# tyiannak/pyAudioAnalysis

Measured on AMD Instinct MI355X. Metric: short-term frames/sec (34-feat, 16 kHz, 50 ms/25 ms) + HBM GB/s vs peak, higher is better.
Workload: dtype f64

## Files before the change

### pyaudioanalysis_amd/csrc/device_common.hpp

```cpp
#pragma once
#include <float.h>
#include <hip/hip_runtime.h>
#include <stdint.h>

namespace paa {

constexpr int kWave = 64;
constexpr int kBase = 34;
constexpr int kFlush = 8;
constexpr double kEps = 2.220446049250313e-16;
#ifdef PAA_EXPERIMENTS
#define PAA_DEBUG_BIT(word, bit) (((word) & (bit)) != 0)
#else
#define PAA_DEBUG_BIT(word, bit) false
#endif

struct ClipDev {
    long long sample_off;
    long long n;
    long long out_off;
    int T;
    int stat_first;
    int stat_count;
    int pad;
// ... 173 lines not shown
    return v;
}
__device__ __forceinline__ int group_min_i(int v) {
    v = min(v, dpp_mov_i<PAA_DPP_X1>(v));
    v = min(v, dpp_mov_i<PAA_DPP_X2>(v));
    v = min(v, dpp_mov_i<PAA_DPP_HM>(v));
    v = min(v, dpp_mov_i<PAA_DPP_RM>(v));
    return v;
}
__device__ __forceinline__ double group_scan_incl(double v) {
    v += dpp_mov<0x111>(v);
    v += dpp_mov<0x112>(v);
    v += dpp_mov<0x114>(v);
    v += dpp_mov<0x118>(v);
    return v;
}

__device__ __forceinline__ void wsync() {
    asm volatile("" ::: "memory");
    __builtin_amdgcn_wave_barrier();
    asm volatile("" ::: "memory");
}


__device__ __forceinline__ double readlane63(double v) {
    const int lo = __builtin_amdgcn_readlane(__double2loint(v), 63);
    const int hi = __builtin_amdgcn_readlane(__double2hiint(v), 63);
    return __hiloint2double(hi, lo);
}
template <int CTRL, int ROWMASK>
__device__ __forceinline__ double dpp_mov_rows(double v) {
    int lo = __builtin_amdgcn_update_dpp(0, __double2loint(v), CTRL, ROWMASK, 0xF, false);
    int hi = __builtin_amdgcn_update_dpp(0, __double2hiint(v), CTRL, ROWMASK, 0xF, false);
    return __hiloint2double(hi, lo);
}
__device__ __forceinline__ double wsum(double v) {
    v = group_sum(v);
    v += dpp_mov_rows<0x142, 0xA>(v);
    v += dpp_mov_rows<0x143, 0xC>(v);
    return readlane63(v);
}
__device__ __forceinline__ double wmax_nonneg(double v) {
    v = group_max(v);
    v = fmax(v, dpp_mov_rows<0x142, 0xA>(v));
    v = fmax(v, dpp_mov_rows<0x143, 0xC>(v));
    return readlane63(v);
}
__device__ __forceinline__ int wsum_i(int v) {
    v = group_sum_i(v);
    v += __builtin_amdgcn_update_dpp(0, v, 0x142, 0xA, 0xF, false);
    v += __builtin_amdgcn_update_dpp(0, v, 0x143, 0xC, 0xF, false);
    return __builtin_amdgcn_readlane(v, 63);
}
__device__ __forceinline__ int wmin_i(int v) {
#pragma unroll
    for (int o = 32; o > 0; o >>= 1) v = min(v, __shfl_xor(v, o, 64));
    return v;
}
__device__ __forceinline__ double wscan_incl(double v) {
    v = group_scan_incl(v);
    v += dpp_mov_rows<0x142, 0xA>(v);
    v += dpp_mov_rows<0x143, 0xC>(v);
    return v;
}

__device__ __forceinline__ double fast_sqrt(double x) {
    const double y = __builtin_amdgcn_rsq(x);
    double g = x * y;
    double h = 0.5 * y;
    const double r = fma(-h, g, 0.5);
    g = fma(g, r, g);
    h = fma(h, r, h);
    const double d = fma(-g, g, x);
    g = fma(d, h, g);
    return (x > 0.0) ? g : 0.0;
}
__device__ __forceinline__ double mag_sqrt(double x) {
    const unsigned hi_ = max((unsigned)__double2hiint(x), 0x01a56e1fu);
    const double y = __builtin_amdgcn_rsq(__hiloint2double((int)hi_, __double2loint(x)));
    const double g = x * y;
    const double h = 0.5 * y;
    const double r = fma(-h, g, 0.5);
    return fma(g, r, g);
}

__device__ __forceinline__ double fast_div(double a, double b) {
    double r = __builtin_amdgcn_rcp(b);
    r = fma(fma(-b, r, 1.0), r, r);
    r = fma(fma(-b, r, 1.0), r, r);
    const double q = a * r;
    return fma(fma(-b, q, a), r, q);
}

__device__ __forceinline__ double fast_log2(double x) {
    double m = __builtin_amdgcn_frexp_mant(x);
    int e = __builtin_amdgcn_frexp_exp(x);
    const bool lo = m < 0.70710678118654752440;
    m = lo ? m + m : m;
    e = lo ? e - 1 : e;
    const double num = m - 1.0, den = m + 1.0;
    double r = __builtin_amdgcn_rcp(den);
    r = fma(fma(-den, r, 1.0), r, r);
    r = fma(fma(-den, r, 1.0), r, r);
    double s = num * r;
    s = fma(fma(-den, s, num), r, s);
    const double z = s * s;
    double p = 1.0 / 21.0;
    p = fma(p, z, 1.0 / 19.0);
    p = fma(p, z, 1.0 / 17.0);
    p = fma(p, z, 1.0 / 15.0);
    p = fma(p, z, 1.0 / 13.0);
    p = fma(p, z, 1.0 / 11.0);
    p = fma(p, z, 1.0 / 9.0);
    p = fma(p, z, 1.0 / 7.0);
    p = fma(p, z, 1.0 / 5.0);
    p = fma(p, z, 1.0 / 3.0);
    p = fma(p, z, 1.0);
    return fma(s * p, 2.8853900817779268147, (double)e);
}
__device__ __forceinline__ double fast_log10(double x) { return fast_log2(x) * 0.30102999566398119521; }

template <typename T> __device__ __forceinline__ double load_sample(const T *p);
template <> __device__ __forceinline__ double load_sample<int16_t>(const int16_t *p) { return (double)(*p); }
template <> __device__ __forceinline__ double load_sample<double>(const double *p) { return *p; }
struct alignas(4) stereo16 { int16_t l, r; };
__device__ __forceinline__ int stereo_word_sum(int w) { return (int)(short)(w & 0xffff) + (w >> 16); }
template <> __device__ __forceinline__ double load_sample<stereo16>(const stereo16 *p) {
    return (double)stereo_word_sum(*reinterpret_cast<const int *>(p));
}
template <typename T> __host__ __device__ constexpr double sample_scale() { return 1.0 / 32768.0; }
template <> __host__ __device__ constexpr double sample_scale<stereo16>() { return 1.0 / 65536.0; }

struct SignRule {
    int zb1, lo, sh;
};
__device__ __forceinline__ int sgn1(int x, const SignRule &q) {
    int t;
    asm("v_med3_i32 %0, %1, %2, 2" : "=v"(t) : "v"(x - q.zb1), "v"(q.lo));
    return t;
}
__device__ __forceinline__ int sgn1(double d) { return ((d > 0.0) ? 2 : 1) - ((d < 0.0) ? 1 : 0); }
__device__ __forceinline__ void sad_acc(int &acc, int a, int b) { asm("v_sad_u32 %0, %1, %2, %0" : "+v"(acc) : "v"(a), "v"(b)); }
template <typename T>
__device__ __forceinline__ SignRule sign_rule(double mean) {
    const double thr = mean * (1.0 / sample_scale<T>());
    const double fl = floor(thr);
    const bool whole = (fl == thr);
    SignRule q;
    q.zb1 = (int)fl - 1;
    q.lo = whole ? 0 : 1;
    q.sh = __builtin_amdgcn_readfirstlane(whole ? 0 : 1);
    asm volatile("" : "+v"(q.zb1), "+v"(q.lo));
    return q;
}

template <typename SumT, typename MmT>
__device__ __forceinline__ ClipNorm clip_norm_wave(const ClipDev &cd, const SumT *__restrict__ psum,
                                                   const MmT *__restrict__ pmin, const MmT *__restrict__ pmax, double sc,
                                                   int window, int lane) {
    SumT s = 0;
    double mn = DBL_MAX, mx = -DBL_MAX;
    const SumT *ps = psum + cd.stat_first;
    const MmT *pn = pmin + cd.stat_first, *px = pmax + cd.stat_first;
    int i = lane;
    for (; i + 192 < cd.stat_count; i += 256) {
        SumT a[4];
// ... 65 lines not shown
```

### pyaudioanalysis_amd/csrc/kernels_fast.hpp

```cpp
#pragma once
#include <algorithm>
#include <vector>

#include "device_common.hpp"
#include "tables.hpp"

namespace paa {

struct FastTables {
    void *d_blob = nullptr;
};
namespace f800 {
struct TabLayout {
    int off_w0, off_k0, off_w1, off_k1, off_w2, off_k2;
    int off_chw, off_chk;
    int off_dct;
    int off_tw2, off_twp;
    int off_sync;
    int melN0, melN1, melN2, chN;
    int mel_clamp;
    double f0, rf0, r_half_fs, f0sq;
    int fixed_lists;
    int pace_mode;
    int total;
// ... 24 lines not shown
constexpr int CH_STRIDE = 12;

template <int S, int NW = 4>
struct Geo {
    static_assert(S % CHUNK == 0 && S % 8 == 0, "step must be a multiple of the 40-sample chunk");
    static constexpr int RAW_N = (QUAD - 1) * S + W;
    static constexpr int NCHUNK = RAW_N / CHUNK;
    static constexpr int CPF = S / CHUNK;
    static constexpr int NPRE = (RAW_N / 8 + 63) / 64;
    static constexpr int PAD = (NW == 8 && S == 800) ? 0 : RAW_PAD;
    static constexpr int RAW_BYTES = (RAW_N + 2 * PAD) * 2;
    static constexpr bool ALIAS = (NW == 8);
    static constexpr int OFF_SPEC = 0;
    static constexpr int OFF_RAW = OFF_SPEC + 5 * NF * 8;
    static constexpr int OFF_CE = ALIAS ? OFF_RAW : OFF_RAW + RAW_BYTES;
    static constexpr int OFF_CZ = OFF_CE + NCHUNK * 8;
    static constexpr int OFF_FV = OFF_CZ + 2 * NCHUNK * 4;
    static constexpr int LDS_BYTES = ALIAS ? OFF_FV : OFF_FV + QUAD * FV_STRIDE * 8;
    static constexpr int WAVE_BYTES = ((LDS_BYTES + 15) / 16) * 16;
    static_assert(OFF_RAW % 16 == 0 && OFF_CE % 8 == 0 && OFF_FV % 8 == 0, "LDS alignment");
    static_assert(QUAD * 40 * 8 <= RAW_BYTES, "msp alias fits in the raw buffer");
    static_assert(!ALIAS || RAW_BYTES <= 2 * NF * 8, "raw[] fits in two spectrum slots");
    static_assert(!ALIAS || QUAD * 40 * 8 + QUAD * FV_STRIDE * 8 <= NF * 8, "msp + fv fit in one spectrum slot");
};

__device__ __forceinline__ void dft5r(double2 &a0, double2 &a1, double2 &a2, double2 &a3, double2 &a4) {
    const double c1 = 0.30901699437494742410;
    const double s1 = 0.95105651629515357212, s2 = 0.58778525229247312917;
    const double2 t1 = cadd(a1, a4), t2 = cadd(a2, a3), t3 = csub(a1, a4), t4 = csub(a2, a3);
    const double2 d = csub(t1, t2);
    const double2 h1 = make_double2(fma(-0.5, t1.x, a0.x), fma(-0.5, t1.y, a0.y));
    const double2 h2 = make_double2(fma(-0.5, t2.x, a0.x), fma(-0.5, t2.y, a0.y));
    const double2 m1 = make_double2(fma(c1, d.x, h2.x), fma(c1, d.y, h2.y));
    const double2 m2 = make_double2(fma(-c1, d.x, h1.x), fma(-c1, d.y, h1.y));
    const double2 n1 = make_double2(fma(s2, t4.x, s1 * t3.x), fma(s2, t4.y, s1 * t3.y));
    const double2 n2 = make_double2(fma(-s1, t4.x, s2 * t3.x), fma(-s1, t4.y, s2 * t3.y));
    a0 = make_double2(a0.x + t1.x + t2.x, a0.y + t1.y + t2.y);
    a1 = sub_i(m1, n1);
    a4 = add_i(m1, n1);
    a2 = sub_i(m2, n2);
    a3 = add_i(m2, n2);
}
__device__ __forceinline__ void dft4r(double2 &a0, double2 &a1, double2 &a2, double2 &a3) {
    const double2 t0 = cadd(a0, a2), t1 = csub(a0, a2), t2 = cadd(a1, a3), t3 = csub(a1, a3);
    a0 = cadd(t0, t2);
    a2 = csub(t0, t2);
    a1 = sub_i(t1, t3);
    a3 = add_i(t1, t3);
}
template <int SERIAL>
__device__ __forceinline__ void dft25_tail(double2 *v);
template <int SERIAL = 0>
__device__ __forceinline__ void dft25(double2 *v) {
#pragma unroll
    for (int r2 = 0; r2 < 5; ++r2) {
        dft5r(v[r2], v[5 + r2], v[10 + r2], v[15 + r2], v[20 + r2]);
        if (SERIAL) __builtin_amdgcn_sched_barrier(0);
    }
    dft25_tail<SERIAL>(v);
}
template <int SERIAL>
__device__ __forceinline__ void dft25_tail(double2 *v) {
#pragma unroll
    for (int q1 = 1; q1 < 5; ++q1)
#pragma unroll
        for (int r2 = 1; r2 < 5; ++r2) {
            const int m = r2 * q1;
            const double cr = (m == 1) ? 0.96858316112863108 : (m == 2) ? 0.87630668004386358 : (m == 3) ? 0.72896862742141155
                            : (m == 4) ? 0.53582679497899666 : (m == 6) ? 0.06279051952931337 : (m == 8) ? -0.42577929156507272
                            : (m == 9) ? -0.63742398974868975 : (m == 12) ? -0.99211470131447788 : -0.63742398974868975;
            const double ci = (m == 1) ? -0.24868988716485479 : (m == 2) ? -0.48175367410171532 : (m == 3) ? -0.68454710592868873
                            : (m == 4) ? -0.84432792550201508 : (m == 6) ? -0.99802672842827156 : (m == 8) ? -0.90482705246601958
                            : (m == 9) ? -0.77051324277578925 : (m == 12) ? -0.12533323356430426 : 0.77051324277578925;
            v[5 * q1 + r2] = cmul(v[5 * q1 + r2], make_double2(cr, ci));
        }
    if (SERIAL) __builtin_amdgcn_sched_barrier(0);
#pragma unroll
    for (int q1 = 0; q1 < 5; ++q1) {
        dft5r(v[5 * q1], v[5 * q1 + 1], v[5 * q1 + 2], v[5 * q1 + 3], v[5 * q1 + 4]);
        if (SERIAL) __builtin_amdgcn_sched_barrier(0);
    }
}
#define PAA_DFT25_POS(q) (5 * ((q) % 5) + (q) / 5)

__device__ __forceinline__ void dft5r_first(int w0, int w1, int w2, int w3, int w4, int m, double2 &a0, double2 &a1,
                                            double2 &a2, double2 &a3, double2 &a4) {
    const double c1 = 0.30901699437494742410;
    const double s1 = 0.95105651629515357212, s2 = 0.58778525229247312917;
    const int x0r = (int)(short)(w0 & 0xffff), x0i = w0 >> 16, x1r = (int)(short)(w1 & 0xffff), x1i = w1 >> 16;
    const int x2r = (int)(short)(w2 & 0xffff), x2i = w2 >> 16, x3r = (int)(short)(w3 & 0xffff), x3i = w3 >> 16;
    const int x4r = (int)(short)(w4 & 0xffff), x4i = w4 >> 16;
    const int m2 = 2 * m;
    const int t1r = x1r + x4r - m2, t1i = x1i + x4i - m2, t2r = x2r + x3r - m2, t2i = x2i + x3i - m2;
    const int t3r = x1r - x4r, t3i = x1i - x4i, t4r = x2r - x3r, t4i = x2i - x3i;
    const int b0r = x0r - m, b0i = x0i - m;
    const double2 D = make_double2((double)(t1r - t2r), (double)(t1i - t2i));
    const double2 H1 = make_double2(0.5 * (double)(2 * b0r - t1r), 0.5 * (double)(2 * b0i - t1i));
    const double2 H2 = make_double2(0.5 * (double)(2 * b0r - t2r), 0.5 * (double)(2 * b0i - t2i));
    const double2 T3 = make_double2((double)t3r, (double)t3i), T4 = make_double2((double)t4r, (double)t4i);
    const double2 M1 = make_double2(fma(c1, D.x, H2.x), fma(c1, D.y, H2.y));
    const double2 M2 = make_double2(fma(-c1, D.x, H1.x), fma(-c1, D.y, H1.y));
    const double2 N1 = make_double2(fma(s2, T4.x, s1 * T3.x), fma(s2, T4.y, s1 * T3.y));
    const double2 N2 = make_double2(fma(-s1, T4.x, s2 * T3.x), fma(-s1, T4.y, s2 * T3.y));
    a0 = make_double2((double)(b0r + t1r + t2r), (double)(b0i + t1i + t2i));
    a1 = sub_i(M1, N1);
    a4 = add_i(M1, N1);
    a2 = sub_i(M2, N2);
    a3 = add_i(M2, N2);
}
template <int SERIAL>
__device__ __forceinline__ void dft25_packed(const int *w, int m, double2 *v) {
#pragma unroll
    for (int r2 = 0; r2 < 5; ++r2) {
        dft5r_first(w[r2], w[5 + r2], w[10 + r2], w[15 + r2], w[20 + r2], m, v[r2], v[5 + r2], v[10 + r2], v[15 + r2], v[20 + r2]);
        if (SERIAL) __builtin_amdgcn_sched_barrier(0);
    }
    dft25_tail<SERIAL>(v);
}

template <int SERIAL = 0>
__device__ __forceinline__ void dft16(double2 *v) {
    const double c = 0.92387953251128676, s = 0.38268343236508977, h = 0.70710678118654752;
#pragma unroll
    for (int r2 = 0; r2 < 4; ++r2) {
        dft4r(v[r2], v[4 + r2], v[8 + r2], v[12 + r2]);
        if (SERIAL) __builtin_amdgcn_sched_barrier(0);
    }
    v[5] = cmul(v[5], make_double2(c, -s));
    v[6] = make_double2(h * (v[6].x + v[6].y), h * (v[6].y - v[6].x));
    v[7] = cmul(v[7], make_double2(s, -c));
    v[9] = make_double2(h * (v[9].x + v[9].y), h * (v[9].y - v[9].x));
    v[10] = make_double2(v[10].y, -v[10].x);
    v[11] = make_double2(h * (v[11].y - v[11].x), -h * (v[11].x + v[11].y));
    v[13] = cmul(v[13], make_double2(s, -c));
    v[14] = make_double2(h * (v[14].y - v[14].x), -h * (v[14].x + v[14].y));
    v[15] = cmul(v[15], make_double2(-c, s));
    if (SERIAL) __builtin_amdgcn_sched_barrier(0);
#pragma unroll
    for (int q1 = 0; q1 < 4; ++q1) {
        dft4r(v[4 * q1], v[4 * q1 + 1], v[4 * q1 + 2], v[4 * q1 + 3]);
        if (SERIAL) __builtin_amdgcn_sched_barrier(0);
    }
}
#define PAA_DFT16_POS(q) (4 * ((q) % 4) + (q) / 4)

__device__ __forceinline__ double dpp_bcast15(double v) { return group_max(v); }


__device__ __forceinline__ double uni(double v) {
    const unsigned long long b = __double_as_longlong(v);
    const unsigned lo = __builtin_amdgcn_readfirstlane((unsigned)b), hi = __builtin_amdgcn_readfirstlane((unsigned)(b >> 32));
    return __longlong_as_double(((unsigned long long)hi << 32) | lo);
}
__device__ __forceinline__ int uni(int v) { return __builtin_amdgcn_readfirstlane(v); }

#ifdef PAA_F800_TIMING
static __device__ unsigned long long g_phase_cycles[16];
static __device__ unsigned long long g_wave_trace[4096 * 4];
#define PAA_T0() unsigned long long t_prev_ = __builtin_readcyclecounter(); unsigned long long t_acc_[12] = {0,0,0,0,0,0,0,0,0,0,0,0}; \
    const unsigned long long t_rt0_ = __builtin_amdgcn_s_memrealtime(), t_c0_ = t_prev_;
#define PAA_TICK(idx) { const unsigned long long t_now_ = __builtin_readcyclecounter(); t_acc_[idx] += t_now_ - t_prev_; t_prev_ = t_now_; }
#define PAA_TEND() if (lane == 0) { for (int z_ = 0; z_ < 12; ++z_) atomicAdd(&g_phase_cycles[z_], t_acc_[z_]); atomicAdd(&g_phase_cycles[15], 1ULL); \
    if (tile_id < 4096) { g_wave_trace[4 * tile_id] = t_rt0_; g_wave_trace[4 * tile_id + 1] = __builtin_amdgcn_s_memrealtime(); \
        g_wave_trace[4 * tile_id + 2] = __builtin_readcyclecounter() - t_c0_; \
        g_wave_trace[4 * tile_id + 3] = (unsigned long long)__builtin_amdgcn_s_getreg((31 << 11) | 4) | ((unsigned long long)__builtin_amdgcn_s_getreg((31 << 11) | 20) << 32); } }
#elif defined(PAA_F800_TRACE)
static __device__ unsigned long long g_phase_cycles[16];
static __device__ unsigned long long g_wave_trace[4096 * 4];
#define PAA_T0() const unsigned long long t_rt0_ = __builtin_amdgcn_s_memrealtime(), t_c0_ = __builtin_readcyclecounter();
#define PAA_TICK(idx)
#define PAA_TEND() if (lane == 0) { atomicAdd(&g_phase_cycles[15], 1ULL); \
    if (tile_id < 4096) { g_wave_trace[4 * tile_id] = t_rt0_; g_wave_trace[4 * tile_id + 1] = __builtin_amdgcn_s_memrealtime(); \
        g_wave_trace[4 * tile_id + 2] = __builtin_readcyclecounter() - t_c0_; \
        g_wave_trace[4 * tile_id + 3] = (unsigned long long)__builtin_amdgcn_s_getreg((31 << 11) | 4) | ((unsigned long long)__builtin_amdgcn_s_getreg((31 << 11) | 20) << 32); } }
#else
#define PAA_T0()
#define PAA_TICK(idx)
#define PAA_TEND()
#endif
#if defined(PAA_F800_TIMING) || defined(PAA_F800_TRACE)
#define PAA_PHASE_READER(NAME)                                                                                          \
    int NAME(unsigned long long *acc16, unsigned long long *trace, int max_waves) {                                     \
        unsigned long long host[16], zero[16] = {0};                                                                    \
        if (hipMemcpyFromSymbol(host, HIP_SYMBOL(f800::g_phase_cycles), sizeof(host)) != hipSuccess) return -1;          \
        for (int i = 0; i < 16; ++i) acc16[i] += host[i];                                                               \
        if (hipMemcpyToSymbol(HIP_SYMBOL(f800::g_phase_cycles), zero, sizeof(zero)) != hipSuccess) return -1;            \
        if (!trace) return 0;                                                                                           \
        const int n = max_waves < 4096 ? max_waves : 4096;                                                              \
        if (hipMemcpyFromSymbol(trace, HIP_SYMBOL(f800::g_wave_trace), (size_t)n * 4 * sizeof(unsigned long long)) != hipSuccess) return -1; \
        return n;                                                                                                       \
    }
#else
#define PAA_PHASE_READER(NAME) int NAME(unsigned long long *, unsigned long long *, int) { return 0; }
#endif

__device__ __forceinline__ double sel64(unsigned long long take_a, double a, double b) {
    int lo, hi;
    asm("v_cndmask_b32_e64 %0, %1, %2, %3" : "=v"(lo) : "v"(__double2loint(b)), "v"(__double2loint(a)), "s"(take_a));
    asm("v_cndmask_b32_e64 %0, %1, %2, %3" : "=v"(hi) : "v"(__double2hiint(b)), "v"(__double2hiint(a)), "s"(take_a));
    return __hiloint2double(hi, lo);
}
__device__ __forceinline__ void store_chunk_pieces(double *dst, const double (&o)[8], int vlo, int vhi, int dbg = 0) {
    if (PAA_DEBUG_BIT(dbg, 4) && !(vlo <= 0 && vhi >= 8)) return;
    if (PAA_DEBUG_BIT(dbg, 8) && (vlo <= 0 && vhi >= 8)) return;
    (void)dbg;
    typedef double f64x4 __attribute__((ext_vector_type(4), aligned(32)));
    typedef double f64x2 __attribute__((ext_vector_type(2), aligned(16)));
    if (vlo <= 0 && vhi >= 8) {
        __builtin_nontemporal_store(f64x4{o[0], o[1], o[2], o[3]}, reinterpret_cast<f64x4 *>(dst));
        __builtin_nontemporal_store(f64x4{o[4], o[5], o[6], o[7]}, reinterpret_cast<f64x4 *>(dst + 4));
        return;
    }
#pragma unroll
    for (int b4 = 0; b4 < 8; b4 += 4) {
        if (vlo <= b4 && vhi >= b4 + 4) {
            *reinterpret_cast<f64x4 *>(dst + b4) = f64x4{o[b4], o[b4 + 1], o[b4 + 2], o[b4 + 3]};
        } else {
#pragma unroll
            for (int b2 = b4; b2 < b4 + 4; b2 += 2) {
                if (vlo <= b2 && vhi >= b2 + 2) {
                    *reinterpret_cast<f64x2 *>(dst + b2) = f64x2{o[b2], o[b2 + 1]};
                } else {
                    if (vlo <= b2 && vhi > b2) dst[b2] = o[b2];
                    if (vlo <= b2 + 1 && vhi > b2 + 1) dst[b2 + 1] = o[b2 + 1];
                }
// ... 21 lines not shown
        const unsigned long long m2 = __builtin_amdgcn_ballot_w64((u & 4) != 0), m1 = __builtin_amdgcn_ballot_w64((u & 2) != 0),
                                 m0 = __builtin_amdgcn_ballot_w64((u & 1) != 0);
        double z[7], y[7], o[8];
#pragma unroll
        for (int j = 0; j < 7; ++j) z[j] = sel64(m2, w[(j + 8 > 10) ? 10 : j + 8], w[j + 4]);
#pragma unroll
        for (int j = 0; j < 7; ++j) y[j] = sel64(m1, z[(j + 2 > 6) ? 6 : j + 2], z[j]);
#pragma unroll
        for (int j = 0; j < 7; ++j) o[j] = sel64(m0, y[(j + 1 > 6) ? 6 : j + 1], y[j]);
        o[7] = o[6];
        store_chunk_pieces(row + g, o, lo - g, hi - g, dbg);
    }
}

template <int S, int DELTAS, int FIXED, int NW>
__global__ __launch_bounds__(64 * NW, NW / 4) void st_fast_800_kernel(PlanDev P, TabLayout L,
                                                                     const unsigned char *__restrict__ blob,
                                                                     const int16_t *__restrict__ sig,
                                                                     const ClipDev *__restrict__ clips,
                                                                     const ClipNorm *__restrict__ norms,
                                                                     const Tile *__restrict__ tiles, int n_tiles,
                                                                     double *__restrict__ out) {
    extern __shared__ __attribute__((aligned(16))) unsigned char smem[];
    {
        const int4 *src4 = reinterpret_cast<const int4 *>(blob);
        int4 *dst4 = reinterpret_cast<int4 *>(smem);
        for (int n = threadIdx.x; n < L.total / 16; n += 64 * NW) dst4[n] = src4[n];
    }
    __syncthreads();
    const double *t_melw0 = reinterpret_cast<const double *>(smem + L.off_w0);
    const int *t_melk0 = reinterpret_cast<const int *>(smem + L.off_k0);
    const double *t_melw1 = reinterpret_cast<const double *>(smem + L.off_w1);
    const int *t_melk1 = reinterpret_cast<const int *>(smem + L.off_k1);
    const double *t_melw2 = reinterpret_cast<const double *>(smem + L.off_w2);
    const int *t_melk2 = reinterpret_cast<const int *>(smem + L.off_k2);
    const double *t_chw = reinterpret_cast<const double *>(smem + L.off_chw);
    const int *t_chk = reinterpret_cast<const int *>(smem + L.off_chk);
    const double *t_dct = reinterpret_cast<const double *>(smem + L.off_dct);
    const double2 *t_tw2 = reinterpret_cast<const double2 *>(smem + L.off_tw2);
    const double2 *t_twp = reinterpret_cast<const double2 *>(smem + L.off_twp);

    const int wave = __builtin_amdgcn_readfirstlane(threadIdx.x >> 6);
    const int tile_id = blockIdx.x * NW + wave;
    volatile int *pace = reinterpret_cast<volatile int *>(smem + L.off_sync);
    int partner = wave;
    if (NW == 8) {
        const int my_simd = (int)((__builtin_amdgcn_s_getreg((31 << 11) | 4) >> 4) & 3u);
        if ((threadIdx.x & 63) == 0) {
            pace[wave] = my_simd;
            pace[8 + wave] = (tile_id < n_tiles) ? 0 : 0x7fffffff;
        }
        __syncthreads();
#pragma unroll
        for (int w = 0; w < 8; ++w) partner = (w != wave && pace[w] == my_simd) ? w : partner;
        partner = __builtin_amdgcn_readfirstlane(partner);
    }
    if (tile_id >= n_tiles) return;
    using G = Geo<S, NW>;
    constexpr int RAW_N = G::RAW_N, NCHUNK = G::NCHUNK, CPF = G::CPF;
    unsigned char *wbase = smem + L.total + wave * G::WAVE_BYTES;
    double *spec = reinterpret_cast<double *>(wbase + G::OFF_SPEC);
    int16_t *raw = reinterpret_cast<int16_t *>(wbase + (G::ALIAS ? 0 : G::OFF_RAW));
    double *msp = reinterpret_cast<double *>(wbase + (G::ALIAS ? 0 : G::OFF_RAW));
    double *cE = reinterpret_cast<double *>(wbase + G::OFF_CE);
    int *cZ = reinterpret_cast<int *>(wbase + G::OFF_CZ);
    int *cF = cZ + NCHUNK;
    double *fv = reinterpret_cast<double *>(wbase + (G::ALIAS ? 0 : G::OFF_FV));

    const int lane = threadIdx.x & 63;
    int g = lane >> 4, i = lane & 15;
    PAA_T0()
    const Tile tl = tiles[tile_id];
    const ClipDev c = clips[tl.clip];
    const ClipNorm nm = wave_clip_norm<int16_t>(P, c, norms, tl.clip, lane);
    const int16_t *xc = sig + c.sample_off;
    const long long Tc = c.T;
    double *oc = out + c.out_off;

    const double f0 = L.f0, rf0 = L.rf0, r_half_fs = L.r_half_fs, f0sq = L.f0sq;
    const int m_int = nm.m_int;
    const double delta_mu = nm.delta_mu;
    const double y_scale2 = nm.y_scale2;
    const double mag_scale = nm.mag_scale;
    const double dc_shift = nm.dc_shift;
    const bool mu_whole = nm.mu_whole != 0;
    const short zb1_ = (short)max(nm.zb - 1, -32768);
    const s16x2 zc_b = {zb1_, zb1_};
    const s16x2 zc_lo = mu_whole ? (s16x2){0, 0} : (s16x2){1, 1};
    const s16x2 zc_two = {2, 2};
    const s16x2 zc_one = {1, 1};
    const int zc_shift = mu_whole ? 0 : 1;

    const int r0 = tl.t0, t_end = tl.t0 + tl.cnt;
    constexpr int HALO = DELTAS ? 2 : 1;
    int q0 = r0 >= HALO ? r0 - HALO : 0;
    int slot0 = 2;
    double vlast = 0.0;
    double hold[7] = {0.0, 0.0, 0.0, 0.0, 0.0, 0.0, 0.0};
    double holdd[7] = {0.0, 0.0, 0.0, 0.0, 0.0, 0.0, 0.0};
    bool first_quad = true;
    int n_done = 0;

    int4 pre[G::NPRE];
#pragma unroll
    for (int r = 0; r < G::NPRE; ++r) pre[r] = make_int4(0, 0, 0, 0);
    bool pre_ok;
#define PAA_F800_FETCH(q)                                                                              \
    {                                                                                                  \
        const long long base_ = (long long)(q) * S;                                                    \
        const int16_t *src_ = xc + base_;                                                              \
        pre_ok = ((reinterpret_cast<uintptr_t>(src_) & 15) == 0) && (c.n - base_ >= RAW_N);            \
        if (pre_ok) {                                                                                  \
            const int4 *s4_ = reinterpret_cast<const int4 *>(src_);                                    \
            _Pragma("unroll") for (int r_ = 0; r_ < G::NPRE; ++r_)                                     \
                if (lane + 64 * r_ < RAW_N / 8) pre[r_] = s4_[lane + 64 * r_];                         \
        }                                                                                              \
    }
    if (NW == 4) PAA_F800_FETCH(q0)

    int16_t before_next = 0;
    int16_t before_reg = 0;
    for (;; first_quad = false) {
        if (!first_quad) q0 += QUAD;
        if (q0 >= t_end) break;
        slot0 = (slot0 + 4) % 5;
        if (NW != 4) asm volatile("" : "+v"(g), "+v"(i));
#define PAA_F800_PACE(half_)                                                                           \
        if (NW == 8 && L.pace_mode != 0) {                                                             \
            const int mine_ = 2 * n_done + (half_);                                                    \
            if (lane == 0) pace[8 + wave] = mine_;                                                     \
            const int other_ = __builtin_amdgcn_readfirstlane(pace[8 + partner]);                      \
            const int d_ = mine_ - other_;                                                             \
            if (d_ < 0) __builtin_amdgcn_s_setprio(3);                                                 \
            else if (d_ > 0) __builtin_amdgcn_s_setprio(0);                                            \
            else __builtin_amdgcn_s_setprio(1);                                                        \
        }
        PAA_F800_PACE(0)
        const int pa = i, pb = (i == 0) ? 0 : 25 - i;
        const bool act = i < 13;
        const int itw = min(i, TW_STRIDE - 1), ich = min(i, CH_STRIDE - 1);
        if (G::ALIAS) {
            const int prev_slot = (slot0 + 4) % 5;
            raw = reinterpret_cast<int16_t *>(spec + ((prev_slot <= 2) ? 3 : 0) * NF);
            msp = spec + prev_slot * NF;
            fv = msp + QUAD * 40;
        }
        {
            const long long base = (long long)q0 * S;
            const int16_t *src = xc + base;
            int16_t before = 0;
            if (lane == 0) before = (!first_quad) ? before_next : ((base > 0) ? src[-1] : src[0]);
            if (NW != 4) PAA_F800_FETCH(q0)
            if (pre_ok) {
                int4 *d4 = reinterpret_cast<int4 *>(raw + G::PAD);
#pragma unroll
                for (int r = 0; r < G::NPRE; ++r)
                    if (lane + 64 * r < RAW_N / 8) d4[lane + 64 * r] = pre[r];
            } else {
                const long long avail = c.n - base;
                for (int n = lane; n < RAW_N; n += 64) raw[G::PAD + n] = (n < avail) ? src[n] : (int16_t)0;
            }
            if (G::PAD > 0 && lane == 0) raw[G::PAD - 1] = before;
            before_reg = before;
            if (NW == 4 && q0 + QUAD < t_end) PAA_F800_FETCH(q0 + QUAD)
        }
        wsync();
// ... 2 lines not shown

        for (int ch = lane; ch < NCHUNK; ch += 64) {
            const int4 *p4 = reinterpret_cast<const int4 *>(raw + G::PAD + CHUNK * ch);
            s16x2 sp;
            if (G::PAD == 0 && ch == 0) sp = (s16x2){0, before_reg};
            else sp = __builtin_bit_cast(s16x2, reinterpret_cast<const int *>(raw + G::PAD + CHUNK * ch)[-1]);
            sp = __builtin_elementwise_min(__builtin_elementwise_max(__builtin_elementwise_sub_sat(sp, zc_b), zc_lo), zc_two);
            double sx2 = 0.0;
            int sx = 0;
            int zacc = 0, zfirst = 0;
#pragma unroll
            for (int v4 = 0; v4 < CHUNK / 8; ++v4) {
                const int4 q = p4[v4];
                const int w[4] = {q.x, q.y, q.z, q.w};
#pragma unroll
                for (int h = 0; h < 4; ++h) {
                    const s16x2 cur = __builtin_bit_cast(s16x2, w[h]);
                    const s16x2 sg = __builtin_elementwise_min(__builtin_elementwise_max(__builtin_elementwise_sub_sat(cur, zc_b), zc_lo), zc_two);
                    const unsigned sgw = __builtin_bit_cast(unsigned, sg);
                    const unsigned shw = __builtin_amdgcn_alignbit(sgw, __builtin_bit_cast(unsigned, sp), 16);
                    if (v4 == 0 && h == 0) zfirst = abs((int)(sgw & 0xffffu) - (int)(shw & 0xffffu));
                    asm("v_sad_u16 %0, %1, %2, %0" : "+v"(zacc) : "v"(sgw), "v"(shw));
                    sp = sg;
                    sx2 += (double)(unsigned)__builtin_amdgcn_sdot2(cur, cur, 0, false);
                    sx = __builtin_amdgcn_sdot2(cur, zc_one, sx, false);
                }
            }
            const double mi = nm.mi;
            const double e2 = fma(mi, fma((double)CHUNK, mi, -2.0 * (double)sx), sx2);
            const int s1 = sx - CHUNK * m_int;
            const double e = y_scale2 * fma(delta_mu, fma(-2.0, (double)s1, nm.chunk_dmu), e2);
            cE[ch] = e;
            cZ[ch] = zacc;
            cF[ch] = zfirst;
        }

        PAA_TICK(1)
        double2 v[25];
        {
            const int *r32 = reinterpret_cast<const int *>(raw + G::PAD) + (S / 2) * g + i;
            int w25[25];
#pragma unroll
            for (int r = 0; r < 25; ++r) w25[r] = r32[16 * r];
            dft25_packed<(NW != 4)>(w25, m_int, v);
        }
        wsync();
        PAA_TICK(2)

        double ax[16], ay[16], bx[16], by[16];
        double2 w2[16];
        if (NW == 4) {
#pragma unroll
            for (int r = 1; r < 16; ++r) w2[r] = t_tw2[r * TW_STRIDE + itw];
        }
        {
            double *pl = spec + ((slot0 + g) % 5) * NF;
#pragma unroll
            for (int q = 0; q < 25; ++q) pl[25 * i + q] = v[PAA_DFT25_POS(q)].x;
            wsync();
#pragma unroll
            for (int r = 0; r < 16; ++r) { ax[r] = pl[pa + 25 * r]; bx[r] = pl[pb + 25 * r]; }
            wsync();
#pragma unroll
            for (int q = 0; q < 25; ++q) pl[25 * i + q] = v[PAA_DFT25_POS(q)].y;
            wsync();
#pragma unroll
            for (int r = 0; r < 16; ++r) { ay[r] = pl[pa + 25 * r]; by[r] = pl[pb + 25 * r]; }
            wsync();
        }

        PAA_TICK(3)
        if (act) {
            double2 a[16], b[16];
            a[0] = make_double2(ax[0], ay[0]);
            b[0] = make_double2(bx[0], by[0]);
            double *sp = spec + ((slot0 + g) % 5) * NF;
#define PAA_F800_BIN(q, wpq)                                                                               \
            {                                                                                              \
                const double2 zk = a[PAA_DFT16_POS(q)];                                                    \
                const double2 zb = b[PAA_DFT16_POS((16 - (q)) % 16)];                                      \
                const int k = pa + 25 * (q);                                                               \
                const double2 e = make_double2(zk.x + zb.x, zk.y - zb.y);                                  \
                const double2 o = make_double2(zk.y + zb.y, zb.x - zk.x);                                  \
                const double2 t = cmul((wpq), o);                                                          \
                double xr = e.x + t.x, xi = e.y + t.y;                                                     \
                const double yr = e.x - t.x, yi = e.y - t.y;                                               \
                 \
                const bool dc_ = ((q) == 0) && (i == 0);                                                   \
                xr = dc_ ? xr - dc_shift : xr;                                                             \
                xi = dc_ ? 0.0 : xi;                                                                       \
                const double mk_ = mag_sqrt(fma(xr, xr, xi * xi)) * mag_scale;                             \
                sp[k] = mk_;                                                                               \
                 \
                const double mm_ = mag_sqrt(fma(yr, yr, yi * yi)) * mag_scale;                             \
                if ((q) == 0) sp[dc_ ? 0 : NF - k] = dc_ ? mk_ : mm_;                                      \
                else sp[NF - k] = mm_;                                                                     \
            }
            if (NW == 4) {
#pragma unroll
                for (int r = 1; r < 16; ++r) {
                    a[r] = cmul(make_double2(ax[r], ay[r]), w2[r]);
                    b[r] = cmul(make_double2(bx[r], by[r]), make_double2(w2[r].x, -w2[r].y));
                }
                double2 wp[16];
#pragma unroll
                for (int q = 0; q < 16; ++q) wp[q] = t_twp[q * TW_STRIDE + itw];
                dft16<0>(a);
                dft16<0>(b);
#pragma unroll
                for (int r = 0; r < 16; ++r) asm volatile("" : "+v"(a[r].x), "+v"(a[r].y), "+v"(b[r].x), "+v"(b[r].y));
#pragma unroll
                for (int q = 0; q < 16; ++q) PAA_F800_BIN(q, wp[q])
            } else {
#pragma unroll
                for (int r0 = 1; r0 < 16; r0 += 3) {
                    double2 wg[3];
#pragma unroll
                    for (int u = 0; u < 3; ++u) wg[u] = t_tw2[(r0 + u) * TW_STRIDE + itw];
#pragma unroll
                    for (int u = 0; u < 3; ++u) {
                        a[r0 + u] = cmul(make_double2(ax[r0 + u], ay[r0 + u]), wg[u]);
                        b[r0 + u] = cmul(make_double2(bx[r0 + u], by[r0 + u]), make_double2(wg[u].x, -wg[u].y));
                    }
                    __builtin_amdgcn_sched_barrier(0);
                }
                dft16<1>(a);
                dft16<1>(b);
#pragma unroll
                for (int r = 0; r < 16; ++r) asm volatile("" : "+v"(a[r].x), "+v"(a[r].y), "+v"(b[r].x), "+v"(b[r].y));
#pragma unroll
                for (int q0_ = 0; q0_ < 16; q0_ += 2) {
                    double2 wg[2];
#pragma unroll
                    for (int u = 0; u < 2; ++u) wg[u] = t_twp[(q0_ + u) * TW_STRIDE + itw];
#pragma unroll
                    for (int u = 0; u < 2; ++u) PAA_F800_BIN(q0_ + u, wg[u])
                    __builtin_amdgcn_sched_barrier(0);
                }
            }
#undef PAA_F800_BIN
        }
        wsync();
        ++n_done;
        PAA_F800_PACE(-1)

        PAA_TICK(4)
        const int t = q0 + g;
        const double *cur = spec + ((slot0 + g) % 5) * NF;
        const double *prv = (t == 0) ? cur : spec + ((slot0 + g + 4) % 5) * NF;
        double Xc[25], Xv[25];
#pragma unroll
        for (int m = 0; m < 25; ++m) { Xc[m] = cur[25 * i + m]; Xv[m] = prv[25 * i + m]; }
        if (G::ALIAS) wsync();
        double sXa = 0.0, sXb = 0.0, sMa = 0.0, sMb = 0.0, sVa = 0.0, sVb = 0.0, mx = 0.0;
        double c5[5] = {0.0, 0.0, 0.0, 0.0, 0.0};
#pragma unroll
        for (int m = 0; m < 24; m += 2) {
            const double X0 = Xc[m], X1 = Xc[m + 1];
            sXa += X0; sXb += X1;
            sVa += Xv[m]; sVb += Xv[m + 1];
            sMa = fma((double)m, X0, sMa); sMb = fma((double)(m + 1), X1, sMb);
            c5[m / 5] = fma(X0, X0, c5[m / 5]); c5[(m + 1) / 5] = fma(X1, X1, c5[(m + 1) / 5]);
            mx = fmax(mx, fmax(X0, X1));
        }
        sXa += Xc[24]; sVa += Xv[24]; sMa = fma(24.0, Xc[24], sMa); c5[4] = fma(Xc[24], Xc[24], c5[4]); mx = fmax(mx, Xc[24]);
        const double cs = ((c5[0] + c5[1]) + (c5[2] + c5[3])) + c5[4];
        double pblk;
        {
            const int i7 = i & 7;
            const int kcut = (0x52541535u >> (4 * i7)) & 7;
            const double pL = c5[0] + ((kcut > 1) ? c5[1] : 0.0) + ((kcut > 2) ? c5[2] : 0.0) + ((kcut > 3) ? c5[3] : 0.0) +
                              ((kcut > 4) ? c5[4] : 0.0);
            const double pH = ((kcut > 1) ? 0.0 : c5[1]) + ((kcut > 2) ? 0.0 : c5[2]) + ((kcut > 3) ? 0.0 : c5[3]) +
                              ((kcut > 4) ? 0.0 : c5[4]);
            const double from_prev = dpp_mov<0x111>(pH);
            const double from_next = dpp_mov<0x101>(pL);
            const bool next_joins = (i7 == 0) || (i7 == 2) || (i7 == 5);
            pblk = pL + from_prev + (next_joins ? from_next : 0.0);
        }
        const bool home = ((0xB5u >> (i & 7)) & 1u) != 0;
        const double base_k = (double)(25 * i + 1);
        double sX = sXa + sXb;
        double sIX = f0 * fma(base_k, sX, sMa + sMb);
        double sXp = sVa + sVb;
        sX = group_sum(sX); sXp = group_sum(sXp);
        sIX = group_sum(sIX); mx = group_max(mx);
        const double sXe = sX + (double)NF * kEps;
        sXp += (double)NF * kEps;
        const double run_incl = group_scan_incl(cs);
        const double sP = dpp_bcast15(run_incl);

        const double eblk = (i < 10) ? cE[CPF * g + 2 * i] + cE[CPF * g + 2 * i + 1] : 0.0;
        const double e_tot = group_sum(eblk);
        double ent_f, ent_e;
        {
            const double sf = fast_div(pblk, sP + kEps), se = fast_div(eblk, e_tot + kEps);
            ent_f = group_sum(home ? -(sf * fast_log2(sf + kEps)) : 0.0);
            ent_e = group_sum((i < 10) ? -(se * fast_log2(se + kEps)) : 0.0);
        }
        int zc = cZ[CPF * g + i] + ((i < 4) ? cZ[CPF * g + 16 + i] : 0) - ((i == 0) ? cF[CPF * g] : 0);
        zc = group_sum_i(zc) << zc_shift;

        PAA_TICK(5)
        const double r = (mx == 0.0) ? 1.0 / kEps : fast_div(1.0, mx);
        const double den = sX * r + kEps;
        const double rden = fast_div(1.0, den);
        const double cen = (sIX * r) * rden;
        const double rX = fast_div(1.0, sXe), rXp = fast_div(1.0, sXp);
        const double cb = base_k - cen * rf0;
        double sSa = 0.0, sSb = 0.0, sFa = 0.0, sFb = 0.0;
#pragma unroll
        for (int m = 0; m < 24; m += 2) {
            const double d0 = cb + (double)m, d1 = cb + (double)(m + 1);
            sSa = fma(d0 * d0, Xc[m], sSa);
            sSb = fma(d1 * d1, Xc[m + 1], sSb);
            const double f0d = Xc[m] * rX - Xv[m] * rXp, f1d = Xc[m + 1] * rX - Xv[m + 1] * rXp;
            sFa = fma(f0d, f0d, sFa);
            sFb = fma(f1d, f1d, sFb);
        }
        {
            const double d0 = cb + 24.0;
            sSa = fma(d0 * d0, Xc[24], sSa);
            const double f0d = Xc[24] * rX - Xv[24] * rXp;
            sFa = fma(f0d, f0d, sFa);
        }
        double sSp = (sSa + sSb) * (f0sq * r), sFl = sFa + sFb;
        sSp = group_sum(sSp);
        sFl = group_sum(sFl);
        const double spread = fast_sqrt(sSp * rden);

        int below = 0;
        {
            const double thr = 0.90 * sP;
            double run = run_incl - cs;
#pragma unroll
            for (int m = 0; m < 25; ++m) {
                run = fma(Xc[m], Xc[m], run);
                below += (run + kEps > thr) ? 0 : 1;
            }
        }
        const int first = group_min_i((below < 25) ? 25 * i + below : 0x7fffffff);

        PAA_TICK(6)
        double *mg = msp + 40 * g;
        {
            double acc0 = 0.0, acc1 = 0.0, acc2 = 0.0;
            const int lo0 = t_melk0[i], lo1 = t_melk1[i], lo2 = t_melk2[i];
#define PAA_MEL_CLASS(acc, lo, N, tw, IDX, UNROLL)                                                      \
            UNROLL for (int n = 0; n < (N); n += 8) {                                                   \
                double xv_[8], wv_[8];                                                                  \
                _Pragma("unroll") for (int u = 0; u < 8; ++u) {                                         \
                    xv_[u] = cur[IDX((lo) + n + u)];                                                    \
                    wv_[u] = (tw)[(n + u) * 16 + i];                                                    \
                }                                                                                       \
                double ea_ = 0.0, eb_ = 0.0;                                                            \
                _Pragma("unroll") for (int u = 0; u < 8; u += 2) {                                      \
                    ea_ = fma(xv_[u], wv_[u], ea_);                                                     \
                    eb_ = fma(xv_[u + 1], wv_[u + 1], eb_);                                             \
                }                                                                                       \
                acc += ea_ + eb_;                                                                       \
            }
#define PAA_IDX_CLAMP(k) min((k), NF - 1)
#define PAA_IDX_PLAIN(k) (k)
            if (FIXED) {
                PAA_MEL_CLASS(acc0, lo0, 8, t_melw0, PAA_IDX_PLAIN, _Pragma("unroll"))
                PAA_MEL_CLASS(acc1, lo1, 16, t_melw1, PAA_IDX_PLAIN, _Pragma("unroll"))
                PAA_MEL_CLASS(acc2, lo2, 16, t_melw2, PAA_IDX_PLAIN, _Pragma("unroll"))
            } else if (L.mel_clamp) {
                PAA_MEL_CLASS(acc0, lo0, L.melN0, t_melw0, PAA_IDX_CLAMP, )
                PAA_MEL_CLASS(acc1, lo1, L.melN1, t_melw1, PAA_IDX_CLAMP, )
                PAA_MEL_CLASS(acc2, lo2, L.melN2, t_melw2, PAA_IDX_CLAMP, )
            } else {
                PAA_MEL_CLASS(acc0, lo0, L.melN0, t_melw0, PAA_IDX_PLAIN, )
                PAA_MEL_CLASS(acc1, lo1, L.melN1, t_melw1, PAA_IDX_PLAIN, )
                PAA_MEL_CLASS(acc2, lo2, L.melN2, t_melw2, PAA_IDX_PLAIN, )
            }
#undef PAA_IDX_CLAMP
#undef PAA_IDX_PLAIN
#undef PAA_MEL_CLASS
            acc2 += dpp_mov<0x128>(acc2);
            mg[i] = fast_log10(acc0 + kEps);
            mg[16 + i] = fast_log10(acc1 + kEps);
            const double l2 = fast_log10(acc2 + kEps);
            if (i < 8) mg[32 + i] = l2;
        }
        PAA_TICK(7)
        double chroma = 0.0;
        {
            const int ch_len = FIXED ? 8 : L.chN;
            for (int n = 0; n < ch_len; n += 8) {
                int kv[8];
                double wv[8], xv[8];
#pragma unroll
                for (int u = 0; u < 8; ++u) { kv[u] = t_chk[(n + u) * CH_STRIDE + ich]; wv[u] = t_chw[(n + u) * CH_STRIDE + ich]; }
#pragma unroll
                for (int u = 0; u < 8; ++u) xv[u] = cur[kv[u]];
#pragma unroll
                for (int u = 0; u < 8; ++u) chroma = fma(xv[u] * xv[u], wv[u], chroma);
            }
            chroma = (sP == 0.0) ? chroma / kEps : fast_div(chroma, sP);
            if (i >= 12) chroma = 0.0;
        }
        wsync();
        PAA_TICK(8)
        double *fg = fv + FV_STRIDE * g;
        if (i < 13) {
            const double *dm = t_dct + 41 * i;
            double c0 = 0.0, c1 = 0.0, c2 = 0.0, c3 = 0.0;
#pragma unroll
// ... 198 lines not shown
```

Baseline: 535.0 million.

## Fuse twiddles into FFT butterflies, fold magnitude scale, expand spread moments

Twiddle multiplications for the radix-16 and radix-25 stages are folded into FMA-based butterflies (x=a+w*o, y=2a-x), so the separate complex multiply and add/sub steps collapse into fused operations. The magnitude scale is folded into the Newton step of the sqrt approximation. Spectral spread is computed from precomputed moments (sum X, sum mX, sum m^2 X) instead of a second per-bin loop. Together these cut FP64 instruction count in the hot per-frame path, at the cost of slightly different rounding behaviour and possible cancellation in the expanded spread formula.

```diff
diff --git a/pyaudioanalysis_amd/csrc/device_common.hpp b/pyaudioanalysis_amd/csrc/device_common.hpp
--- a/pyaudioanalysis_amd/csrc/device_common.hpp
+++ b/pyaudioanalysis_amd/csrc/device_common.hpp
@@ -279,6 +279,12 @@
     const double h = 0.5 * y;
     const double r = fma(-h, g, 0.5);
     return fma(g, r, g);
+}
+__device__ __forceinline__ double mag_sqrt_scaled(double x, double c1, double c2) {
+    const unsigned hi_ = max((unsigned)__double2hiint(x), 0x01a56e1fu);
+    const double y = __builtin_amdgcn_rsq(__hiloint2double((int)hi_, __double2loint(x)));
+    const double g = x * y;
+    return g * fma(g, y * c1, c2);
 }
 
 __device__ __forceinline__ double fast_div(double a, double b) {
diff --git a/pyaudioanalysis_amd/csrc/kernels_fast.hpp b/pyaudioanalysis_amd/csrc/kernels_fast.hpp
--- a/pyaudioanalysis_amd/csrc/kernels_fast.hpp
+++ b/pyaudioanalysis_amd/csrc/kernels_fast.hpp
@@ -130,6 +130,53 @@
     }
 }
 #define PAA_DFT25_POS(q) (5 * ((q) % 5) + (q) / 5)
+
+__device__ __forceinline__ void tw_butterfly(double2 &a, double2 &x, double2 w) {
+    const double2 p = make_double2(fma(w.x, x.x, fma(-w.y, x.y, a.x)), fma(w.x, x.y, fma(w.y, x.x, a.y)));
+    x = make_double2(fma(2.0, a.x, -p.x), fma(2.0, a.y, -p.y));
+    a = p;
+}
+__device__ __forceinline__ void dft5r_sums(double2 &a0, double2 t1, double2 t2, double2 t3, double2 t4, double2 &a1,
+                                           double2 &a2, double2 &a3, double2 &a4) {
+    const double c1 = 0.30901699437494742410;
+    const double s1 = 0.95105651629515357212, s2 = 0.58778525229247312917;
+    const double2 d = csub(t1, t2);
+    const double2 h1 = make_double2(fma(-0.5, t1.x, a0.x), fma(-0.5, t1.y, a0.y));
+    const double2 h2 = make_double2(fma(-0.5, t2.x, a0.x), fma(-0.5, t2.y, a0.y));
+    const double2 m1 = make_double2(fma(c1, d.x, h2.x), fma(c1, d.y, h2.y));
+    const double2 m2 = make_double2(fma(-c1, d.x, h1.x), fma(-c1, d.y, h1.y));
+    const double2 n1 = make_double2(fma(s2, t4.x, s1 * t3.x), fma(s2, t4.y, s1 * t3.y));
+    const double2 n2 = make_double2(fma(-s1, t4.x, s2 * t3.x), fma(-s1, t4.y, s2 * t3.y));
+    a0 = make_double2(a0.x + t1.x + t2.x, a0.y + t1.y + t2.y);
+    a1 = sub_i(m1, n1);
+    a4 = add_i(m1, n1);
+    a2 = sub_i(m2, n2);
+    a3 = add_i(m2, n2);
+}
+__device__ __forceinline__ double2 w25_const(int m) {
+    const double cr = (m == 1) ? 0.96858316112863108 : (m == 2) ? 0.87630668004386358 : (m == 3) ? 0.72896862742141155
+                    : (m == 4) ? 0.53582679497899666 : (m == 6) ? 0.06279051952931337 : (m == 8) ? -0.42577929156507272
+                    : (m == 9) ? -0.63742398974868975 : (m == 12) ? -0.99211470131447788 : -0.63742398974868975;
+    const double ci = (m == 1) ? -0.24868988716485479 : (m == 2) ? -0.48175367410171532 : (m == 3) ? -0.68454710592868873
+                    : (m == 4) ? -0.84432792550201508 : (m == 6) ? -0.99802672842827156 : (m == 8) ? -0.90482705246601958
+                    : (m == 9) ? -0.77051324277578925 : (m == 12) ? -0.12533323356430426 : 0.77051324277578925;
+    return make_double2(cr, ci);
+}
+template <int SERIAL>
+__device__ __forceinline__ void dft25_tail_tw(double2 *v) {
+    dft5r(v[0], v[1], v[2], v[3], v[4]);
+    if (SERIAL) __builtin_amdgcn_sched_barrier(0);
+#pragma unroll
+    for (int q1 = 1; q1 < 5; ++q1) {
+        double2 *u = v + 5 * q1;
+        double2 t1 = cmul(u[1], w25_const(q1)), t3 = u[4];
+        double2 t2 = cmul(u[2], w25_const(2 * q1)), t4 = u[3];
+        tw_butterfly(t1, t3, w25_const(4 * q1));
+        tw_butterfly(t2, t4, w25_const(3 * q1));
+        dft5r_sums(u[0], t1, t2, t3, t4, u[1], u[2], u[3], u[4]);
+        if (SERIAL) __builtin_amdgcn_sched_barrier(0);
+    }
+}
 
 __device__ __forceinline__ void dft5r_first(int w0, int w1, int w2, int w3, int w4, int m, double2 &a0, double2 &a1,
                                             double2 &a2, double2 &a3, double2 &a4) {
@@ -163,17 +210,23 @@
         dft5r_first(w[r2], w[5 + r2], w[10 + r2], w[15 + r2], w[20 + r2], m, v[r2], v[5 + r2], v[10 + r2], v[15 + r2], v[20 + r2]);
         if (SERIAL) __builtin_amdgcn_sched_barrier(0);
     }
-    dft25_tail<SERIAL>(v);
-}
-
+    dft25_tail_tw<SERIAL>(v);
+}
+
+template <int SERIAL>
+__device__ __forceinline__ void dft16_tail(double2 *v);
 template <int SERIAL = 0>
 __device__ __forceinline__ void dft16(double2 *v) {
-    const double c = 0.92387953251128676, s = 0.38268343236508977, h = 0.70710678118654752;
 #pragma unroll
     for (int r2 = 0; r2 < 4; ++r2) {
         dft4r(v[r2], v[4 + r2], v[8 + r2], v[12 + r2]);
         if (SERIAL) __builtin_amdgcn_sched_barrier(0);
     }
+    dft16_tail<SERIAL>(v);
+}
+template <int SERIAL>
+__device__ __forceinline__ void dft16_tail(double2 *v) {
+    const double c = 0.92387953251128676, s = 0.38268343236508977, h = 0.70710678118654752;
     v[5] = cmul(v[5], make_double2(c, -s));
     v[6] = make_double2(h * (v[6].x + v[6].y), h * (v[6].y - v[6].x));
     v[7] = cmul(v[7], make_double2(s, -c));
@@ -189,6 +242,33 @@
         dft4r(v[4 * q1], v[4 * q1 + 1], v[4 * q1 + 2], v[4 * q1 + 3]);
         if (SERIAL) __builtin_amdgcn_sched_barrier(0);
     }
+}
+template <int SERIAL, typename TwF>
+__device__ __forceinline__ void dft16_tw_pair(double2 *a, double2 *b, TwF tw) {
+#pragma unroll
+    for (int r2 = 0; r2 < 4; ++r2) {
+        const double2 w1 = tw(4 + r2), w2 = tw(8 + r2), w3 = tw(12 + r2);
+        const double2 w0 = (r2 == 0) ? make_double2(1.0, 0.0) : tw(r2);
+        const double2 w0c = make_double2(w0.x, -w0.y), w1c = make_double2(w1.x, -w1.y);
+        const double2 w2c = make_double2(w2.x, -w2.y), w3c = make_double2(w3.x, -w3.y);
+        double2 a0 = (r2 == 0) ? a[0] : cmul(a[r2], w0), a1 = cmul(a[4 + r2], w1), a2 = a[8 + r2], a3 = a[12 + r2];
+        double2 b0 = (r2 == 0) ? b[0] : cmul(b[r2], w0c), b1 = cmul(b[4 + r2], w1c), b2 = b[8 + r2], b3 = b[12 + r2];
+        tw_butterfly(a0, a2, w2);
+        tw_butterfly(a1, a3, w3);
+        tw_butterfly(b0, b2, w2c);
+        tw_butterfly(b1, b3, w3c);
+        a[r2] = cadd(a0, a1);
+        a[8 + r2] = csub(a0, a1);
+        a[4 + r2] = sub_i(a2, a3);
+        a[12 + r2] = add_i(a2, a3);
+        b[r2] = cadd(b0, b1);
+        b[8 + r2] = csub(b0, b1);
+        b[4 + r2] = sub_i(b2, b3);
+        b[12 + r2] = add_i(b2, b3);
+        if (SERIAL) __builtin_amdgcn_sched_barrier(0);
+    }
+    dft16_tail<SERIAL>(a);
+    dft16_tail<SERIAL>(b);
 }
 #define PAA_DFT16_POS(q) (4 * ((q) % 4) + (q) / 4)
 
@@ -376,6 +456,7 @@
     const double delta_mu = nm.delta_mu;
     const double y_scale2 = nm.y_scale2;
     const double mag_scale = nm.mag_scale;
+    const double mag_c1 = uni(-0.5 * mag_scale), mag_c2 = uni(1.5 * mag_scale);
     const double dc_shift = nm.dc_shift;
     const bool mu_whole = nm.mu_whole != 0;
     const short zb1_ = (short)max(nm.zb - 1, -32768);
@@ -544,50 +625,37 @@
                 const int k = pa + 25 * (q);                                                               \
                 const double2 e = make_double2(zk.x + zb.x, zk.y - zb.y);                                  \
                 const double2 o = make_double2(zk.y + zb.y, zb.x - zk.x);                                  \
-                const double2 t = cmul((wpq), o);                                                          \
-                double xr = e.x + t.x, xi = e.y + t.y;                                                     \
-                const double yr = e.x - t.x, yi = e.y - t.y;                                               \
+                             \
+                const double2 w_ = (wpq);                                                                  \
+                double xr = fma(w_.x, o.x, fma(-w_.y, o.y, e.x)), xi = fma(w_.x, o.y, fma(w_.y, o.x, e.y)); \
+                const double yr = fma(2.0, e.x, -xr), yi = fma(2.0, e.y, -xi);                             \
                  \
                 const bool dc_ = ((q) == 0) && (i == 0);                                                   \
                 xr = dc_ ? xr - dc_shift : xr;                                                             \
                 xi = dc_ ? 0.0 : xi;                                                                       \
-                const double mk_ = mag_sqrt(fma(xr, xr, xi * xi)) * mag_scale;                             \
+                const double mk_ = mag_sqrt_scaled(fma(xr, xr, xi * xi), mag_c1, mag_c2);                 \
                 sp[k] = mk_;                                                                               \
                  \
-                const double mm_ = mag_sqrt(fma(yr, yr, yi * yi)) * mag_scale;                             \
+                const double mm_ = mag_sqrt_scaled(fma(yr, yr, yi * yi), mag_c1, mag_c2);                 \
                 if ((q) == 0) sp[dc_ ? 0 : NF - k] = dc_ ? mk_ : mm_;                                      \
                 else sp[NF - k] = mm_;                                                                     \
             }
+#pragma unroll
+            for (int r = 1; r < 16; ++r) {
+                a[r] = make_double2(ax[r], ay[r]);
+                b[r] = make_double2(bx[r], by[r]);
+            }
             if (NW == 4) {
-#pragma unroll
-                for (int r = 1; r < 16; ++r) {
-                    a[r] = cmul(make_double2(ax[r], ay[r]), w2[r]);
-                    b[r] = cmul(make_double2(bx[r], by[r]), make_double2(w2[r].x, -w2[r].y));
-                }
                 double2 wp[16];
 #pragma unroll
                 for (int q = 0; q < 16; ++q) wp[q] = t_twp[q * TW_STRIDE + itw];
-                dft16<0>(a);
-                dft16<0>(b);
+                dft16_tw_pair<0>(a, b, [&](int r) { return w2[r]; });
 #pragma unroll
                 for (int r = 0; r < 16; ++r) asm volatile("" : "+v"(a[r].x), "+v"(a[r].y), "+v"(b[r].x), "+v"(b[r].y));
 #pragma unroll
                 for (int q = 0; q < 16; ++q) PAA_F800_BIN(q, wp[q])
             } else {
-#pragma unroll
-                for (int r0 = 1; r0 < 16; r0 += 3) {
-                    double2 wg[3];
-#pragma unroll
-                    for (int u = 0; u < 3; ++u) wg[u] = t_tw2[(r0 + u) * TW_STRIDE + itw];
-#pragma unroll
-                    for (int u = 0; u < 3; ++u) {
-                        a[r0 + u] = cmul(make_double2(ax[r0 + u], ay[r0 + u]), wg[u]);
-                        b[r0 + u] = cmul(make_double2(bx[r0 + u], by[r0 + u]), make_double2(wg[u].x, -wg[u].y));
-                    }
-                    __builtin_amdgcn_sched_barrier(0);
-                }
-                dft16<1>(a);
-                dft16<1>(b);
+                dft16_tw_pair<1>(a, b, [&](int r) { return t_tw2[r * TW_STRIDE + itw]; });
 #pragma unroll
                 for (int r = 0; r < 16; ++r) asm volatile("" : "+v"(a[r].x), "+v"(a[r].y), "+v"(b[r].x), "+v"(b[r].y));
 #pragma unroll
@@ -614,7 +682,7 @@
 #pragma unroll
         for (int m = 0; m < 25; ++m) { Xc[m] = cur[25 * i + m]; Xv[m] = prv[25 * i + m]; }
         if (G::ALIAS) wsync();
-        double sXa = 0.0, sXb = 0.0, sMa = 0.0, sMb = 0.0, sVa = 0.0, sVb = 0.0, mx = 0.0;
+        double sXa = 0.0, sXb = 0.0, sMa = 0.0, sMb = 0.0, sQa = 0.0, sQb = 0.0, sVa = 0.0, sVb = 0.0, mx = 0.0;
         double c5[5] = {0.0, 0.0, 0.0, 0.0, 0.0};
 #pragma unroll
         for (int m = 0; m < 24; m += 2) {
@@ -622,10 +690,11 @@
             sXa += X0; sXb += X1;
             sVa += Xv[m]; sVb += Xv[m + 1];
             sMa = fma((double)m, X0, sMa); sMb = fma((double)(m + 1), X1, sMb);
+            sQa = fma((double)(m * m), X0, sQa); sQb = fma((double)((m + 1) * (m + 1)), X1, sQb);
             c5[m / 5] = fma(X0, X0, c5[m / 5]); c5[(m + 1) / 5] = fma(X1, X1, c5[(m + 1) / 5]);
             mx = fmax(mx, fmax(X0, X1));
         }
-        sXa += Xc[24]; sVa += Xv[24]; sMa = fma(24.0, Xc[24], sMa); c5[4] = fma(Xc[24], Xc[24], c5[4]); mx = fmax(mx, Xc[24]);
+        sXa += Xc[24]; sVa += Xv[24]; sMa = fma(24.0, Xc[24], sMa); sQa = fma(576.0, Xc[24], sQa); c5[4] = fma(Xc[24], Xc[24], c5[4]); mx = fmax(mx, Xc[24]);
         const double cs = ((c5[0] + c5[1]) + (c5[2] + c5[3])) + c5[4];
         double pblk;
         {
@@ -643,7 +712,8 @@
         const bool home = ((0xB5u >> (i & 7)) & 1u) != 0;
         const double base_k = (double)(25 * i + 1);
         double sX = sXa + sXb;
-        double sIX = f0 * fma(base_k, sX, sMa + sMb);
+        const double sXl = sX, sMl = sMa + sMb;
+        double sIX = f0 * fma(base_k, sX, sMl);
         double sXp = sVa + sVb;
         sX = group_sum(sX); sXp = group_sum(sXp);
         sIX = group_sum(sIX); mx = group_max(mx);
@@ -670,23 +740,19 @@
         const double cen = (sIX * r) * rden;
         const double rX = fast_div(1.0, sXe), rXp = fast_div(1.0, sXp);
         const double cb = base_k - cen * rf0;
-        double sSa = 0.0, sSb = 0.0, sFa = 0.0, sFb = 0.0;
+        double sFa = 0.0, sFb = 0.0;
 #pragma unroll
         for (int m = 0; m < 24; m += 2) {
-            const double d0 = cb + (double)m, d1 = cb + (double)(m + 1);
-            sSa = fma(d0 * d0, Xc[m], sSa);
-            sSb = fma(d1 * d1, Xc[m + 1], sSb);
             const double f0d = Xc[m] * rX - Xv[m] * rXp, f1d = Xc[m + 1] * rX - Xv[m + 1] * rXp;
             sFa = fma(f0d, f0d, sFa);
             sFb = fma(f1d, f1d, sFb);
         }
         {
-            const double d0 = cb + 24.0;
-            sSa = fma(d0 * d0, Xc[24], sSa);
             const double f0d = Xc[24] * rX - Xv[24] * rXp;
             sFa = fma(f0d, f0d, sFa);
         }
-        double sSp = (sSa + sSb) * (f0sq * r), sFl = sFa + sFb;
+        const double sSl = fma(cb, fma(cb, sXl, 2.0 * sMl), sQa + sQb);
+        double sSp = sSl * (f0sq * r), sFl = sFa + sFb;
         sSp = group_sum(sSp);
         sFl = group_sum(sFl);
         const double spread = fast_sqrt(sSp * rden);
```

New measurement: 558.4 million (median of 6 runs). 1.04x the previous value.
